# risc0/zeth

Hardware: AMD Instinct MI355X
Metric: segments/sec (higher is better)
Workload: dtype u32

## Files before the change

### zeth_amd/csrc/hash.hip

```cpp
#include "common.h"
#include "image_tree.h"
#include "poseidon2.h"
#include "poseidon2_wide.h"

using namespace zkh;

static_assert(zkh::ZKH_P2_PTAB == zkh::P2_TAB_WORDS, "common.h ZKH_P2_PTAB must equal poseidon2.h P2_TAB_WORDS");

namespace {

__global__ __launch_bounds__(256, 4) void k_hash_rows(uint32_t* __restrict__ out, const uint32_t* __restrict__ matrix,
                                                   size_t rows, uint32_t cols, const uint32_t* __restrict__ rc,
                                                   const uint32_t* __restrict__ diag) {
    const size_t r = (size_t)blockIdx.x * blockDim.x + threadIdx.x;
    if (r >= rows) return;
    uint32_t s[CELLS];
#pragma unroll
    for (int i = 0; i < CELLS; i++) s[i] = 0;
    const uint32_t* src = matrix + r;
    const uint32_t full = cols / RATE, tail = cols % RATE;
    const uint32_t blocks = full + (tail || cols == 0 ? 1u : 0u);
    for (uint32_t b = 0; b < blocks; b++) {
        const uint32_t* bsrc = src + (size_t)b * RATE * rows;
        if (b < full) {
#pragma unroll
            for (int i = 0; i < RATE; i++) s[i] = bsrc[(size_t)i * rows];
        } else {
#pragma unroll
            for (int i = 0; i < RATE; i++) s[i] = (uint32_t)i < tail ? bsrc[(size_t)i * rows] : 0u;
        }
        poseidon2_mix_sponge(s, rc, diag, b + 1 == blocks);
#pragma unroll
        for (int i = RATE; i < CELLS; i++) s[i] = p2_signed(s[i]);
    }
#pragma unroll
    for (int i = 0; i < OUT; i++) s[i] = canon((int32_t)s[RATE + i]);
    uint4* o = (uint4*)(out + r * 8);
    o[0] = make_uint4(s[0], s[1], s[2], s[3]);
    o[1] = make_uint4(s[4], s[5], s[6], s[7]);
}

__device__ __forceinline__ void fold_one(uint32_t* __restrict__ io, size_t input_size, size_t output_size, size_t i,
                                         const uint32_t* __restrict__ rc, const uint32_t* __restrict__ diag) {
    const uint4* src = (const uint4*)(io + (input_size + 2 * i) * 8);
    uint32_t s[CELLS];
    const uint4 a = src[0], b = src[1], c = src[2], d = src[3];
    s[0] = a.x; s[1] = a.y; s[2] = a.z; s[3] = a.w; s[4] = b.x; s[5] = b.y; s[6] = b.z; s[7] = b.w;
    s[8] = c.x; s[9] = c.y; s[10] = c.z; s[11] = c.w; s[12] = d.x; s[13] = d.y; s[14] = d.z; s[15] = d.w;
#pragma unroll
    for (int k = RATE; k < CELLS; k++) s[k] = 0;
    poseidon2_mix_raw<0, OUT, RATE>(s, rc, diag);
#pragma unroll
    for (int k = 0; k < OUT; k++) s[k] = p2_finish(s[k]);
    uint4* o = (uint4*)(io + (output_size + i) * 8);
    o[0] = make_uint4(s[0], s[1], s[2], s[3]);
    o[1] = make_uint4(s[4], s[5], s[6], s[7]);
}
__global__ __launch_bounds__(256, 4) void k_hash_fold(uint32_t* __restrict__ io, size_t input_size, size_t output_size,
                                                   const uint32_t* __restrict__ rc, const uint32_t* __restrict__ diag) {
    const size_t i = (size_t)blockIdx.x * blockDim.x + threadIdx.x;
    if (i >= output_size) return;
    fold_one(io, input_size, output_size, i, rc, diag);
}
__global__ __launch_bounds__(256, 4) void k_hash_fold_list(uint32_t* __restrict__ io, size_t width, const uint32_t* __restrict__ list,
                                                        const uint32_t* __restrict__ count, const uint32_t* __restrict__ rc,
                                                        const uint32_t* __restrict__ diag) {
    const uint32_t t = blockIdx.x * blockDim.x + threadIdx.x;
    if (t >= *count) return;
    fold_one(io, 2 * width, width, list[t], rc, diag);
}
__global__ __launch_bounds__(256, 4) void k_hash_walk(const uint32_t* __restrict__ list, const uint32_t* __restrict__ from, const uint32_t* __restrict__ sib,
                                                   const uint32_t* __restrict__ count, const uint32_t* __restrict__ proof, const uint32_t* __restrict__ off,
                                                   const uint32_t* __restrict__ cur, uint32_t* __restrict__ next, const uint32_t* __restrict__ rc,
                                                   const uint32_t* __restrict__ diag) {
    const uint32_t lane = blockIdx.x * blockDim.x + threadIdx.x, r = lane >> 1, v = lane & 1;
    if (r >= *count) return;
    const uint32_t item = from[r], clean = sib[r];
    const uint32_t* mine = cur + 16 * (size_t)item + 8 * v;
    const uint32_t* other = clean == 0xffffffffu ? mine + 16 : proof + *off + 8 * (size_t)clean;
    const bool odd = clean != 0xffffffffu && (list[item] & 1);
    const uint32_t* left = odd ? other : mine;
    const uint32_t* right = odd ? mine : other;
    uint32_t s[CELLS];
#pragma unroll
    for (int k = 0; k < 8; k++) { s[k] = left[k]; s[8 + k] = right[k]; }
#pragma unroll
    for (int k = RATE; k < CELLS; k++) s[k] = 0;
    poseidon2_mix_raw<0, OUT, RATE>(s, rc, diag);
#pragma unroll
    for (int k = 0; k < OUT; k++) s[k] = p2_finish(s[k]);
    uint4* o = (uint4*)(next + 16 * (size_t)r + 8 * v);
    o[0] = make_uint4(s[0], s[1], s[2], s[3]);
    o[1] = make_uint4(s[4], s[5], s[6], s[7]);
}

__device__ __forceinline__ void wide_fold_one(uint32_t* __restrict__ io, size_t input_size, size_t output_size, uint32_t gid,
                                              const uint32_t* rcs, const uint32_t* __restrict__ pc) {
    const uint32_t j = gid & 7;
    size_t parent = gid >> 3;
    const bool live = parent < output_size;
    if (!live) parent = output_size - 1;
    uint32_t c[4] = {0, 0, 0, 0};
    if (j < 4) {
        const uint4 v = *(const uint4*)(io + (input_size + 2 * parent) * 8 + 4 * j);
        c[0] = v.x; c[1] = v.y; c[2] = v.z; c[3] = v.w;
    }
    wide_permute(c, j, rcs, pc);
    if (live && j < 2) *(uint4*)(io + (output_size + parent) * 8 + 4 * j) = make_uint4(c[0], c[1], c[2], c[3]);
}
constexpr int TAIL_LOG = 7;
__global__ __launch_bounds__(8 << TAIL_LOG) void k_hash_fold_subtree(uint32_t* __restrict__ io, size_t first_parents, uint32_t levels,
                                                                     const uint32_t* __restrict__ rc, const uint32_t* __restrict__ pc) {
    __shared__ __attribute__((aligned(16))) uint32_t rcs[ROUNDS_TOTAL * CELLS + 8];
    for (uint32_t w = threadIdx.x; w < ROUNDS_TOTAL * CELLS; w += blockDim.x) rcs[w] = rc[w];
    __syncthreads();
    for (uint32_t l = 0; l < levels; l++) {
        const size_t parents = first_parents >> l;
        const uint32_t local = (1u << TAIL_LOG) >> l;
        if ((threadIdx.x >> 6) * 8 < local) {
            const uint32_t grp = threadIdx.x >> 3;
            const uint32_t gid = grp < local ? (uint32_t)((blockIdx.x * local + grp) * 8 + (threadIdx.x & 7)) : 0xffffffffu;
            wide_fold_one(io, 2 * parents, parents, gid, rcs, pc);
        }
        __threadfence_block();
        __syncthreads();
    }
}
__global__ __launch_bounds__(8 << TAIL_LOG) void k_hash_fold_tail(uint32_t* __restrict__ io, size_t first_parents,
                                                                  const uint32_t* __restrict__ rc, const uint32_t* __restrict__ pc) {
    __shared__ __attribute__((aligned(16))) uint32_t rcs[ROUNDS_TOTAL * CELLS + 8];
    for (uint32_t w = threadIdx.x; w < ROUNDS_TOTAL * CELLS; w += blockDim.x) rcs[w] = rc[w];
    __syncthreads();
    for (size_t parents = first_parents; parents >= 1; parents >>= 1) {
        if ((threadIdx.x >> 6) * 8 < parents)
            wide_fold_one(io, 2 * parents, parents, threadIdx.x, rcs, pc);
        __threadfence_block();
        __syncthreads();
    }
}

__global__ __launch_bounds__(256) void k_poseidon2_mix(uint32_t* __restrict__ io, size_t count, const uint32_t* __restrict__ rc,
                                                       const uint32_t* __restrict__ diag) {
    const size_t i = (size_t)blockIdx.x * blockDim.x + threadIdx.x;
    if (i >= count) return;
    uint4* p = (uint4*)(io + i * CELLS);
    uint32_t s[CELLS];
#pragma unroll
    for (int q = 0; q < CELLS / 4; q++) { const uint4 v = p[q]; s[4 * q] = v.x; s[4 * q + 1] = v.y; s[4 * q + 2] = v.z; s[4 * q + 3] = v.w; }
    poseidon2_mix(s, rc, diag);
#pragma unroll
    for (int q = 0; q < CELLS / 4; q++) p[q] = make_uint4(s[4 * q], s[4 * q + 1], s[4 * q + 2], s[4 * q + 3]);
}

}

extern "C" const char* zkh_poseidon2_mix(zkh_ctx* c, zkh_buf* states, size_t count) {
    ZKH_REQUIRE(states && states->len == count * CELLS, "poseidon2_mix: buffer is not count x 24 words");
    if (!count) return nullptr;
    bind_thread(c);
    k_poseidon2_mix<<<(unsigned)((count + 255) / 256), 256, 0, c->stream>>>(states->ptr(), count, c->tab.rc, c->tab.diag);
    return last_launch_error("poseidon2_mix");
}
extern "C" const char* zkh_hash_rows(zkh_ctx* c, zkh_buf* out, const zkh_buf* matrix) {
    ZKH_REQUIRE(out->len % 8 == 0 && out->len, "hash_rows: output is not a digest array");
    const size_t rows = out->len / 8;
    ZKH_REQUIRE(matrix->len % rows == 0, "hash_rows: matrix size %zu not a multiple of rows %zu", matrix->len, rows);
    const size_t cols = matrix->len / rows;
    ProfScope prof(c, "hash_rows", 4.0 * matrix->len + 32.0 * rows);
    k_hash_rows<<<(unsigned)((rows + 255) / 256), 256, 0, c->stream>>>(out->ptr(), matrix->ptr(), rows, (uint32_t)cols,
                                                                      c->tab.rc, c->tab.diag);
    return last_launch_error("hash_rows");
}
extern "C" const char* zkh_hash_fold(zkh_ctx* c, zkh_buf* io, size_t input_size, size_t output_size) {
    ZKH_REQUIRE(io->len % 8 == 0, "hash_fold: not a digest array");
    ZKH_REQUIRE((input_size + 2 * output_size) * 8 <= io->len && output_size * 2 <= input_size, "hash_fold: ranges out of bounds");
    if (!output_size) return nullptr;
    ProfScope prof(c, "hash_fold", 96.0 * output_size);
    k_hash_fold<<<(unsigned)((output_size + 255) / 256), 256, 0, c->stream>>>(io->ptr(), input_size, output_size, c->tab.rc,
                                                                             c->tab.diag);
    return last_launch_error("hash_fold");
}
extern "C" const char* zkh_merkle_fold_all(zkh_ctx* c, zkh_buf* nodes, size_t rows) {
    ZKH_REQUIRE(nodes->len == rows * 16 && rows && (rows & (rows - 1)) == 0, "merkle_fold_all: nodes must hold 2*rows digests");
    return merkle_fold_from(c, nodes, rows);
}
extern "C" const char* zkh_merkle_build(zkh_ctx* c, zkh_buf* nodes, const zkh_buf* matrix, size_t rows) {
    ZKH_REQUIRE(nodes && matrix && nodes->len == rows * 16 && rows && (rows & (rows - 1)) == 0, "merkle_build: nodes must hold 2*rows digests");
    ZKH_REQUIRE(matrix->len % rows == 0, "merkle_build: matrix size %zu not a multiple of rows %zu", matrix->len, rows);
    zkh_buf* leaves = nullptr;
    ZKH_TRY(zkh_slice(nodes, rows * 8, rows * 8, &leaves));
    const char* err = zkh_hash_rows(c, leaves, matrix);
    zkh_release(leaves);
    ZKH_TRY(err);
    return merkle_fold_from(c, nodes, rows);
}
const char* zkh::merkle_fold_from(zkh_ctx* c, zkh_buf* nodes, size_t first_layer) {
    for (size_t layer = first_layer; layer >= 2; layer /= 2) {
        const size_t parents = layer / 2;
        if (parents > ((size_t)1 << WIDE_LOG)) {
            ZKH_TRY(zkh_hash_fold(c, nodes, layer, parents));
        } else if (parents > ((size_t)1 << TAIL_LOG)) {
            uint32_t levels = 0;
            while ((parents >> levels) > ((size_t)1 << TAIL_LOG)) levels++;
            ProfScope prof(c, "hash_fold_wide", 96.0 * (2 * parents - (parents >> (levels - 1))));
            k_hash_fold_subtree<<<(unsigned)(parents >> TAIL_LOG), 8 << TAIL_LOG, 0, c->stream>>>(nodes->ptr(), parents, levels, c->tab.rc,
                                                                                                   c->tab.diag);
            ZKH_TRY(last_launch_error("hash_fold_wide"));
            layer >>= (levels - 1);
        } else {
            ProfScope prof(c, "hash_fold_tail", 96.0 * (2 * parents - 1));
            k_hash_fold_tail<<<1, 8 << TAIL_LOG, 0, c->stream>>>(nodes->ptr(), parents, c->tab.rc, c->tab.diag);
            ZKH_TRY(last_launch_error("hash_fold_tail"));
            break;
        }
    }
    return nullptr;
}
const char* zkh::hash_fold_listed(zkh_ctx* c, zkh_buf* nodes, size_t width, const uint32_t* list, const uint32_t* count, uint32_t bound) {
    ZKH_REQUIRE(bound && bound <= width && 32 * width <= nodes->len, "hash_fold_listed: %u parents of %zu in %zu words", bound, width, nodes->len);
    ProfScope prof(c, "image_sparse", 100.0 * bound);
    k_hash_fold_list<<<(bound + 255) / 256, 256, 0, c->stream>>>(nodes->ptr(), width, list, count, c->tab.rc, c->tab.diag);
    return last_launch_error("image_sparse");
}
const char* zkh::hash_walk_layer(zkh_ctx* c, const uint32_t* list, const uint32_t* from, const uint32_t* sib, const uint32_t* count, const uint32_t* proof,
                                 const uint32_t* off, const uint32_t* cur, uint32_t* next, uint32_t bound) {
    ZKH_REQUIRE(bound && bound <= 0x7fffffffu, "hash_walk_layer: %u parents", bound);
    ProfScope prof(c, "walk_hash", 200.0 * bound);
    k_hash_walk<<<(unsigned)((2 * (size_t)bound + 255) / 256), 256, 0, c->stream>>>(list, from, sib, count, proof, off, cur, next, c->tab.rc, c->tab.diag);
    return last_launch_error("walk_hash");
}
```

### zeth_amd/csrc/ntt.hip

```cpp
#include "common.h"
#include "ntt_lazy.h"

using namespace zkh;

namespace {

constexpr int NTT_THREADS = 256;

struct PassParams {
    const uint32_t* in;
    uint32_t* out;
    size_t in_col_stride;
    size_t out_col_stride;
    uint32_t log_n;
    uint32_t L, R;
    uint32_t log_t;
    uint32_t expand_bits;
    uint32_t first_layer;
    uint32_t twiddle;
    uint32_t scale;
    uint32_t zk_shift;
    const uint32_t* tile_tw;
    const uint32_t* layer_tw;
    const uint32_t* tw_lo;
    const uint32_t* tw_hi;
    const uint32_t* sh_lo;
    const uint32_t* sh_hi;
    uint32_t tiles_per_col;
    uint32_t lazy;
    uint32_t lazy_comp;
    uint32_t shift16[16];
};

template <bool INVERSE>
__global__ __launch_bounds__(NTT_THREADS) void k_ntt_pass(PassParams p) {
    extern __shared__ __attribute__((aligned(16))) uint32_t tile[];
    const uint32_t T = 1u << p.log_t, rows = 1u << p.R, elems = rows << p.log_t;
    const uint32_t tid = threadIdx.x;
    const uint32_t tile_id = xcd_remap(blockIdx.x, p.tiles_per_col);
    const uint32_t col = blockIdx.y;
    const uint32_t ltiles = 1u << (p.L - p.log_t);
    const uint32_t a = tile_id >> (p.L - p.log_t), lt = tile_id & (ltiles - 1);
    const size_t base = ((size_t)a << (p.L + p.R)) + ((size_t)lt << p.log_t);
    const uint32_t l0 = lt << p.log_t;
    const uint32_t* in = p.in + (size_t)col * p.in_col_stride;
    uint32_t* out = p.out + (size_t)col * p.out_col_stride;
    const uint32_t tw_shift = MAX_LOG_N - (p.L + p.R);
    const uint32_t pad_mask = INVERSE ? 0u : (1u << p.expand_bits) - (1u << (p.first_layer - 1));

    for (uint32_t e = tid; e < elems; e += NTT_THREADS) {
        const uint32_t m = e >> p.log_t, t = e & (T - 1);
        const size_t gi = base + ((size_t)m << p.L) + t;
        uint32_t v = (gi & pad_mask) ? 0u : in[gi >> p.expand_bits];
        if (!INVERSE && p.twiddle) {
            const uint32_t r = __brev(m) >> (32 - p.R);
            const uint32_t ex = ((l0 + t) * r) << tw_shift;
            const uint32_t w = mul_mod(p.tw_lo[ex & (TW_SIZE - 1)], p.tw_hi[ex >> TW_BITS]);
            v = mul_mod(v, w);
        }
        tile[e] = v;
    }
    __syncthreads();

    const uint32_t half_elems = elems >> 1;
    if (INVERSE) {
        for (uint32_t j = p.R; j >= 1; j--) {
            const uint32_t hb = j - 1;
            for (uint32_t q = tid; q < half_elems; q += NTT_THREADS) {
                const uint32_t t = q & (T - 1), mm = q >> p.log_t;
                const uint32_t low = mm & ((1u << hb) - 1), m = ((mm >> hb) << j) | low;
                const uint32_t i0 = (m << p.log_t) | t, i1 = i0 + (1u << (hb + p.log_t));
                const uint32_t x = tile[i0], y = tile[i1];
                const uint32_t w = p.tile_tw[low << (LDS_TW_LOG - j)];
                tile[i0] = add_mod(x, y);
                tile[i1] = mul_mod(x - y + P, w);
            }
            __syncthreads();
        }
    } else {
        for (uint32_t j = p.first_layer; j <= p.R; j++) {
            const uint32_t hb = j - 1;
            for (uint32_t q = tid; q < half_elems; q += NTT_THREADS) {
                const uint32_t t = q & (T - 1), mm = q >> p.log_t;
                const uint32_t low = mm & ((1u << hb) - 1), m = ((mm >> hb) << j) | low;
                const uint32_t i0 = (m << p.log_t) | t, i1 = i0 + (1u << (hb + p.log_t));
                const uint32_t w = p.tile_tw[low << (LDS_TW_LOG - j)];
                const uint32_t x = tile[i0], y = mul_mod(tile[i1], w);
                tile[i0] = add_mod(x, y);
                tile[i1] = sub_mod(x, y);
            }
            __syncthreads();
        }
    }

    for (uint32_t e = tid; e < elems; e += NTT_THREADS) {
        const uint32_t m = e >> p.log_t, t = e & (T - 1);
        const size_t gi = base + ((size_t)m << p.L) + t;
        uint32_t v = tile[e];
        if (INVERSE) {
            if (p.twiddle) {
                const uint32_t r = __brev(m) >> (32 - p.R);
                const uint32_t ex = ((l0 + t) * r) << tw_shift;
                const uint32_t w = mul_mod(p.tw_lo[ex & (TW_SIZE - 1)], p.tw_hi[ex >> TW_BITS]);
                v = mul_mod(v, w);
            }
            if (p.scale) v = mul_mod(v, p.scale);
            if (p.zk_shift) {
                const uint32_t pos = (uint32_t)gi;
                const uint32_t ex = __brev(pos) >> (32 - p.log_n);
                v = mul_mod(v, mul_mod(p.sh_lo[ex & (TW_SIZE - 1)], p.sh_hi[ex >> TW_BITS]));
            }
        }
        out[gi] = v;
    }
}

template <int R, bool INVERSE>
__global__ __launch_bounds__(256) void k_ntt_top(PassParams p) {
    constexpr int N = 1 << R;
    const uint32_t j0 = (blockIdx.x * 256u + threadIdx.x) << 2;
    const uint32_t* in = p.in + (size_t)blockIdx.y * p.in_col_stride + j0;
    uint32_t* out = p.out + (size_t)blockIdx.y * p.out_col_stride + j0;
    const uint32_t tw_shift = MAX_LOG_N - p.log_n;
    uint32_t v[N][4];
#pragma unroll
    for (int m = 0; m < N; m++) {
        const uint4 w = *(const uint4*)(in + ((size_t)m << p.L));
        v[m][0] = w.x; v[m][1] = w.y; v[m][2] = w.z; v[m][3] = w.w;
    }
    auto root = [&](uint32_t e) -> uint32_t {
        const uint32_t ex = e << tw_shift;
        return mul_mod(p.tw_lo[ex & (TW_SIZE - 1)], p.tw_hi[ex >> TW_BITS]);
    };
    auto four_step = [&]() {
        const uint32_t step = root(1u);
        uint32_t g = root(j0);
#pragma unroll
        for (int c = 0; c < 4; c++) {
            uint32_t pw[N];
            pw[1] = g;
#pragma unroll
            for (int r = 2; r < N; r++) pw[r] = mul_mod(pw[r - 1], g);
#pragma unroll
            for (int m = 1; m < N; m++) {
                const int r = (int)(__builtin_bitreverse32((uint32_t)m) >> (32 - R));
                v[m][c] = mul_mod(v[m][c], pw[r]);
            }
            if (c < 3) g = mul_mod(g, step);
        }
    };
    if (!INVERSE) {
        four_step();
#pragma unroll
        for (int j = 1; j <= R; j++) {
            const int hb = j - 1;
#pragma unroll
            for (int i0 = 0; i0 < N; i0++) {
                if (i0 & (1 << hb)) continue;
                const int low = i0 & ((1 << hb) - 1), i1 = i0 + (1 << hb);
                const uint32_t w = low ? p.tile_tw[(uint32_t)low << (LDS_TW_LOG - j)] : 0u;
#pragma unroll
                for (int c = 0; c < 4; c++) {
                    const uint32_t x = v[i0][c], y = low ? mul_mod(v[i1][c], w) : v[i1][c];
                    v[i0][c] = add_mod(x, y);
                    v[i1][c] = sub_mod(x, y);
                }
            }
        }
    } else {
#pragma unroll
        for (int j = R; j >= 1; j--) {
            const int hb = j - 1;
#pragma unroll
            for (int i0 = 0; i0 < N; i0++) {
                if (i0 & (1 << hb)) continue;
                const int low = i0 & ((1 << hb) - 1), i1 = i0 + (1 << hb);
                const uint32_t w = low ? p.tile_tw[(uint32_t)low << (LDS_TW_LOG - j)] : 0u;
#pragma unroll
                for (int c = 0; c < 4; c++) {
                    const uint32_t x = v[i0][c], y = v[i1][c];
                    v[i0][c] = add_mod(x, y);
                    v[i1][c] = low ? mul_mod(x - y + P, w) : sub_mod(x, y);
                }
            }
        }
        four_step();
    }
#pragma unroll
    for (int m = 0; m < N; m++) *(uint4*)(out + ((size_t)m << p.L)) = make_uint4(v[m][0], v[m][1], v[m][2], v[m][3]);
}

__global__ void k_zk_shift(uint32_t* io, size_t total, uint32_t log_n, const uint32_t* sh_lo, const uint32_t* sh_hi) {
    size_t i = (size_t)blockIdx.x * blockDim.x + threadIdx.x;
    if (i >= total) return;
    const uint32_t pos = (uint32_t)(i & (((size_t)1 << log_n) - 1));
    const uint32_t ex = log_n ? __brev(pos) >> (32 - log_n) : 0;
// ... 7 lines not shown
    const uint32_t mid = blockIdx.x;
    const uint32_t rmid = mid_bits ? __brev(mid) >> (32 - mid_bits) : 0;
    if (rmid < mid) return;
    uint32_t* col = io + (size_t)blockIdx.y * col_stride;
    const uint32_t H = 1u << BR_H;
    for (uint32_t e = threadIdx.x; e < H * H; e += blockDim.x) {
        const uint32_t hi = e >> BR_H, lo = e & (H - 1);
        ta[e] = col[((size_t)hi << (log_n - BR_H)) | ((size_t)mid << BR_H) | lo];
        if (rmid != mid) tb[e] = col[((size_t)hi << (log_n - BR_H)) | ((size_t)rmid << BR_H) | lo];
    }
    __syncthreads();
    for (uint32_t e = threadIdx.x; e < H * H; e += blockDim.x) {
        const uint32_t hi2 = e >> BR_H, lo2 = e & (H - 1);
        const uint32_t shi = __brev(lo2) >> (32 - BR_H), slo = __brev(hi2) >> (32 - BR_H);
        const uint32_t src = (shi << BR_H) | slo;
        col[((size_t)hi2 << (log_n - BR_H)) | ((size_t)rmid << BR_H) | lo2] = ta[src];
        if (rmid != mid) col[((size_t)hi2 << (log_n - BR_H)) | ((size_t)mid << BR_H) | lo2] = tb[src];
    }
}
__global__ void k_bit_reverse_small(uint32_t* io, uint32_t log_n, size_t count) {
    size_t g = (size_t)blockIdx.x * blockDim.x + threadIdx.x;
    size_t n = (size_t)1 << log_n;
    if (g >= n * count) return;
    uint32_t i = (uint32_t)(g & (n - 1));
    uint32_t r = log_n ? __brev(i) >> (32 - log_n) : 0;
    if (i < r) {
        uint32_t* col = io + (g - i);
        uint32_t x = col[i], y = col[r];
        col[i] = y; col[r] = x;
    }
}


template <int LOGR, bool INVERSE, bool BASE0, int J_LO, bool LAZY = false>
__device__ __forceinline__ void radix_layers(uint32_t (&v)[1 << LOGR], const uint32_t* __restrict__ ltab,
                                             const uint32_t base_low, const int first_b) {
    constexpr int N = 1 << LOGR;
    if (!INVERSE && LAZY) {
        lazy_layers<LOGR, BASE0, J_LO>(v, ltab, base_low, first_b);
    } else if (INVERSE) {
#pragma unroll
        for (int b = LOGR - 1; b >= 0; b--) {
            const uint32_t* tw = ltab + (1u << (J_LO + b - 1));
#pragma unroll
            for (int kk = 0; kk < (1 << b); kk++) {
                const bool unit = BASE0 && kk == 0;
                const uint32_t w = unit ? 0u : tw[base_low + ((uint32_t)kk << (J_LO - 1))];
#pragma unroll
                for (int hi = 0; hi < (N >> (b + 1)); hi++) {
                    const int k = (hi << (b + 1)) | kk;
                    const uint32_t x = v[k], y = v[k + (1 << b)];
                    v[k] = add_mod(x, y);
                    v[k + (1 << b)] = unit ? sub_mod(x, y) : mul_mod(x - y + P, w);
                }
            }
        }
    } else {
#pragma unroll
        for (int b = 0; b < LOGR; b++) {
            if (b < first_b) continue;
            const uint32_t* tw = ltab + (1u << (J_LO + b - 1));
#pragma unroll
            for (int kk = 0; kk < (1 << b); kk++) {
                const bool unit = BASE0 && kk == 0;
                const uint32_t w = unit ? 0u : tw[base_low + ((uint32_t)kk << (J_LO - 1))];
#pragma unroll
                for (int hi = 0; hi < (N >> (b + 1)); hi++) {
                    const int k = (hi << (b + 1)) | kk;
                    const uint32_t x = v[k], y = unit ? v[k + (1 << b)] : mul_mod(v[k + (1 << b)], w);
                    v[k] = add_mod(x, y);
                    v[k + (1 << b)] = sub_mod(x, y);
                }
            }
        }
    }
}

template <bool INVERSE, bool LAZY = false>
__global__ __launch_bounds__(256) void k_ntt_low12(PassParams p) {
    __shared__ __attribute__((aligned(16))) uint32_t lds[4096];
    const uint32_t tid = threadIdx.x;
    const uint32_t tile = xcd_remap(blockIdx.x, p.tiles_per_col);
    const size_t base = (size_t)tile << 12;
    const uint32_t* in = p.in + (size_t)blockIdx.y * p.in_col_stride;
    uint32_t* out = p.out + (size_t)blockIdx.y * p.out_col_stride;
    const uint32_t* __restrict__ ltab = p.layer_tw;
    const uint32_t hi = tid >> 4, low = tid & 15;
    uint32_t v[16];
    if (INVERSE) {
#pragma unroll
        for (int k = 0; k < 16; k++) v[k] = in[base + k * 256 + tid];
        radix_layers<4, true, false, 9>(v, ltab, tid, 0);
#pragma unroll
        for (int k = 0; k < 16; k++) lds[k * 256 + tid] = v[k];
        __syncthreads();
#pragma unroll
        for (int k = 0; k < 16; k++) v[k] = lds[hi * 256 + k * 16 + low];
        radix_layers<4, true, false, 5>(v, ltab, low, 0);
#pragma unroll
        for (int k = 0; k < 16; k++) lds[hi * 256 + k * 16 + low] = v[k];
        __syncthreads();
#pragma unroll
        for (int q = 0; q < 4; q++) {
            const uint4 w = ((const uint4*)lds)[tid * 4 + q];
            v[4 * q] = w.x; v[4 * q + 1] = w.y; v[4 * q + 2] = w.z; v[4 * q + 3] = w.w;
        }
        radix_layers<4, true, true, 1>(v, ltab, 0, 0);
        const size_t pos0 = base + (size_t)tid * 16;
        if (p.zk_shift) {
            const uint32_t ex = __brev((uint32_t)pos0) >> (32 - p.log_n);
            const uint32_t b = mul_mod(p.sh_lo[ex & (TW_SIZE - 1)], p.sh_hi[ex >> TW_BITS]);
#pragma unroll
            for (int k = 0; k < 16; k++) v[k] = mul_mod(mul_mod(v[k], b), p.shift16[k]);
        } else if (p.scale) {
#pragma unroll
            for (int k = 0; k < 16; k++) v[k] = mul_mod(v[k], p.scale);
        }
#pragma unroll
        for (int q = 0; q < 4; q++) ((uint4*)(out + pos0))[q] = make_uint4(v[4 * q], v[4 * q + 1], v[4 * q + 2], v[4 * q + 3]);
    } else {
        const size_t pos0 = base + (size_t)tid * 16;
        if (p.expand_bits == 0) {
#pragma unroll
            for (int q = 0; q < 4; q++) {
                const uint4 w = ((const uint4*)(in + pos0))[q];
                v[4 * q] = w.x; v[4 * q + 1] = w.y; v[4 * q + 2] = w.z; v[4 * q + 3] = w.w;
            }
        } else if (p.expand_bits == 2) {
            const uint4 w = *(const uint4*)(in + (pos0 >> 2));
            v[0] = v[1] = v[2] = v[3] = w.x; v[4] = v[5] = v[6] = v[7] = w.y;
            v[8] = v[9] = v[10] = v[11] = w.z; v[12] = v[13] = v[14] = v[15] = w.w;
        } else {
#pragma unroll
            for (int k = 0; k < 16; k++) v[k] = in[(pos0 + k) >> p.expand_bits];
        }
        radix_layers<4, false, true, 1, LAZY>(v, ltab, 0, (int)p.expand_bits);
#pragma unroll
        for (int q = 0; q < 4; q++) ((uint4*)lds)[tid * 4 + q] = make_uint4(v[4 * q], v[4 * q + 1], v[4 * q + 2], v[4 * q + 3]);
        __syncthreads();
#pragma unroll
        for (int k = 0; k < 16; k++) v[k] = lds[hi * 256 + k * 16 + low];
        radix_layers<4, false, false, 5, LAZY>(v, ltab, low, 0);
#pragma unroll
        for (int k = 0; k < 16; k++) lds[hi * 256 + k * 16 + low] = v[k];
        __syncthreads();
#pragma unroll
        for (int k = 0; k < 16; k++) v[k] = lds[k * 256 + tid];
        radix_layers<4, false, false, 9, LAZY>(v, ltab, tid, 0);
#pragma unroll
        for (int k = 0; k < 16; k++) out[base + k * 256 + tid] = v[k];
    }
}

template <int RH, bool INVERSE, bool LAZY = false>
__global__ __launch_bounds__(1 << RH) void k_ntt_high(PassParams p) {
    constexpr int LT = 4;
    constexpr uint32_t TW = 1u << LT;
    extern __shared__ __attribute__((aligned(16))) uint32_t lds[];
    const uint32_t tid = threadIdx.x, t = tid & (TW - 1), g = tid >> LT;
    const uint32_t tile_id = xcd_remap(blockIdx.x, p.tiles_per_col), col = blockIdx.y;
    const uint32_t lt_bits = p.L - LT;
    const uint32_t a = tile_id >> lt_bits, lt = tile_id & ((1u << lt_bits) - 1);
    const size_t base = ((size_t)a << (p.L + RH)) + ((size_t)lt << LT);
    const uint32_t lcol = (lt << LT) + t;
    const uint32_t tw_shift = MAX_LOG_N - (p.L + RH);
    const char* in = (const char*)(p.in + (size_t)col * p.in_col_stride + base);
    char* out = (char*)(p.out + (size_t)col * p.out_col_stride + base);
    const uint32_t tb = t * 4u;
#define TILE_IN(row) (*(const uint32_t*)(in + ((((uint32_t)(row)) << (p.L + 2)) + tb)))
#define TILE_OUT(row) (*(uint32_t*)(out + ((((uint32_t)(row)) << (p.L + 2)) + tb)))
    const uint32_t* __restrict__ ltab = p.layer_tw;
    auto tmul = [](uint32_t x, uint32_t y) -> uint32_t {
        return (LAZY && !INVERSE) ? (uint32_t)smont((int32_t)x, (int32_t)y) : mul_mod(x, y);
    };
    auto root = [&](uint32_t e) -> uint32_t {
        const uint32_t ex = e << tw_shift;
        return tmul(p.tw_lo[ex & (TW_SIZE - 1)], p.tw_hi[ex >> TW_BITS]);
    };
    uint32_t tw[16];
    if (RH == 10) {
        uint32_t w0 = root(lcol * (__brev(g) >> 26));
        if (LAZY) w0 = tmul(w0, p.lazy_comp);
        const uint32_t u1 = root(lcol * 64u), v1 = root(lcol * 256u);
        const uint32_t u2 = tmul(u1, u1), u3 = tmul(u2, u1), v2 = tmul(v1, v1), v3 = tmul(v2, v1);
        const uint32_t wi[4] = {w0, tmul(w0, u2), tmul(w0, u1), tmul(w0, u3)};
#pragma unroll
        for (int i = 0; i < 4; i++) {
            tw[4 * i] = wi[i]; tw[4 * i + 1] = tmul(wi[i], v2); tw[4 * i + 2] = tmul(wi[i], v1); tw[4 * i + 3] = tmul(wi[i], v3);
        }
    } else {
        uint32_t w0 = root(lcol * (__brev(g) >> 28));
        if (LAZY) w0 = tmul(w0, p.lazy_comp);
        const uint32_t q1 = root(lcol * 16u);
        uint32_t qp[16];
        qp[0] = w0;
#pragma unroll
        for (int e = 1; e < 16; e++) qp[e] = tmul(qp[e - 1], q1);
#pragma unroll
        for (int k = 0; k < 16; k++) tw[k] = qp[__builtin_bitreverse8((unsigned char)k) >> 4];
    }
    uint32_t v[16];
    if (RH == 10) {
        const uint32_t hi = g >> 2, low = g & 3;
        if (INVERSE) {
#pragma unroll
            for (int k = 0; k < 16; k++) v[k] = TILE_IN(k * 64 + g);
            radix_layers<4, true, false, 7>(v, ltab, g, 0);
#pragma unroll
            for (int k = 0; k < 16; k++) lds[(k * 64 + g) * TW + t] = v[k];
            __syncthreads();
#pragma unroll
            for (int k = 0; k < 16; k++) v[k] = lds[(hi * 64 + k * 4 + low) * TW + t];
            radix_layers<4, true, false, 3>(v, ltab, low, 0);
#pragma unroll
            for (int k = 0; k < 16; k++) lds[(hi * 64 + k * 4 + low) * TW + t] = v[k];
            __syncthreads();
#pragma unroll
            for (int i = 0; i < 4; i++) {
                uint32_t u[4];
                const uint32_t m0 = (g * 4 + i) * 4;
#pragma unroll
                for (int k = 0; k < 4; k++) u[k] = lds[(m0 + k) * TW + t];
                radix_layers<2, true, true, 1>(u, ltab, 0, 0);
#pragma unroll
                for (int k = 0; k < 4; k++) {
                    uint32_t x = mul_mod(u[k], tw[4 * i + k]);
                    if (p.scale) x = mul_mod(x, p.scale);
                    TILE_OUT(m0 + k) = x;
                }
            }
        } else {
#pragma unroll
            for (int i = 0; i < 4; i++) {
                uint32_t u[4];
                const uint32_t m0 = (g * 4 + i) * 4;
#pragma unroll
                for (int k = 0; k < 4; k++) {
                    const uint32_t x = TILE_IN(m0 + k);
                    u[k] = LAZY ? (uint32_t)smont((int32_t)x, (int32_t)tw[4 * i + k]) : mul_mod(x, tw[4 * i + k]);
                }
                radix_layers<2, false, true, 1, LAZY>(u, ltab, 0, 0);
#pragma unroll
                for (int k = 0; k < 4; k++) lds[(m0 + k) * TW + t] = u[k];
            }
            __syncthreads();
#pragma unroll
            for (int k = 0; k < 16; k++) v[k] = lds[(hi * 64 + k * 4 + low) * TW + t];
            radix_layers<4, false, false, 3, LAZY>(v, ltab, low, 0);
#pragma unroll
            for (int k = 0; k < 16; k++) lds[(hi * 64 + k * 4 + low) * TW + t] = v[k];
            __syncthreads();
#pragma unroll
            for (int k = 0; k < 16; k++) v[k] = lds[(k * 64 + g) * TW + t];
            radix_layers<4, false, false, 7, LAZY>(v, ltab, g, 0);
#pragma unroll
            for (int k = 0; k < 16; k++) TILE_OUT(k * 64 + g) = LAZY ? canon((int32_t)v[k]) : v[k];
        }
    } else {
        if (INVERSE) {
#pragma unroll
            for (int k = 0; k < 16; k++) v[k] = TILE_IN(k * 16 + g);
            radix_layers<4, true, false, 5>(v, ltab, g, 0);
#pragma unroll
            for (int k = 0; k < 16; k++) lds[(k * 16 + g) * TW + t] = v[k];
            __syncthreads();
#pragma unroll
            for (int k = 0; k < 16; k++) v[k] = lds[(g * 16 + k) * TW + t];
            radix_layers<4, true, true, 1>(v, ltab, 0, 0);
#pragma unroll
            for (int k = 0; k < 16; k++) {
                uint32_t x = mul_mod(v[k], tw[k]);
                if (p.scale) x = mul_mod(x, p.scale);
                TILE_OUT(g * 16 + k) = x;
            }
        } else {
#pragma unroll
            for (int k = 0; k < 16; k++) {
                const uint32_t x = TILE_IN(g * 16 + k);
                v[k] = LAZY ? (uint32_t)smont((int32_t)x, (int32_t)tw[k]) : mul_mod(x, tw[k]);
            }
            radix_layers<4, false, true, 1, LAZY>(v, ltab, 0, 0);
#pragma unroll
            for (int k = 0; k < 16; k++) lds[(g * 16 + k) * TW + t] = v[k];
            __syncthreads();
#pragma unroll
            for (int k = 0; k < 16; k++) v[k] = lds[(k * 16 + g) * TW + t];
            radix_layers<4, false, false, 5, LAZY>(v, ltab, g, 0);
#pragma unroll
            for (int k = 0; k < 16; k++) TILE_OUT(k * 16 + g) = LAZY ? canon((int32_t)v[k]) : v[k];
        }
    }
}
#undef TILE_IN
#undef TILE_OUT

struct Pass { uint32_t L, R; };
std::vector<Pass> plan_passes(uint32_t log_n) {
    std::vector<Pass> v;
    if (log_n <= 12) { v.push_back({0, log_n}); return v; }
    if (log_n < 18) {
        const uint32_t low = (log_n + 1) / 2;
        v.push_back({0, low});
        v.push_back({low, log_n - low});
        return v;
    }
    const uint32_t rem = log_n - 12;
    v.push_back({0, 12});
    if (rem == 8 || rem == 10 || rem <= 7) v.push_back({12, rem});
    else if (rem == 9) { v.push_back({12, 8}); v.push_back({20, 1}); }
    else if (rem == 11 || rem == 12) { v.push_back({12, 8}); v.push_back({20, rem - 8}); }
    else { v.push_back({12, 10}); v.push_back({22, rem - 10}); }
    return v;
}

const char* run_transform(zkh_ctx* c, bool inverse, const uint32_t* in, size_t in_col_stride, uint32_t* out,
                          size_t out_col_stride, uint32_t log_n, size_t count, uint32_t expand_bits, bool zk, const char* name) {
    ZKH_REQUIRE(log_n <= (uint32_t)MAX_LOG_N, "%s: transform size 2^%u exceeds the supported 2^%d", name, log_n, MAX_LOG_N);
    ZKH_REQUIRE(count <= 65535, "%s: too many columns (%zu)", name, count);
    std::vector<Pass> passes = plan_passes(log_n);
    const size_t n = (size_t)1 << log_n;
    Fp ninv = fp_inv(fp_encode((uint32_t)(n % P)));
    const size_t npass = passes.size();
    const bool lazy = !inverse && npass == 2 && passes[0].R == 12 && (passes[1].R == 8 || passes[1].R == 10) && expand_bits <= 4;
    const uint32_t lazy_reds = lazy ? lazy_reductions(4, expand_bits) + 2 * lazy_reductions(4, 0) + lazy_reductions(passes[1].R, 0) : 0;
    const uint32_t lazy_comp = lazy ? fp_pow(Fp::raw(R2), lazy_reds).v : 0;
    for (size_t pi = 0; pi < npass; pi++) {
        const Pass ps = inverse ? passes[npass - 1 - pi] : passes[pi];
        PassParams p{};
        const bool first = pi == 0, last = pi + 1 == npass;
        p.in = first ? in : out;
        p.in_col_stride = first ? in_col_stride : out_col_stride;
        p.out = out; p.out_col_stride = out_col_stride;
        p.log_n = log_n; p.L = ps.L; p.R = ps.R;
        const bool reg_high = ps.L >= 4 && (ps.R == 8 || ps.R == 10);
        p.log_t = ps.L == 0 ? 0 : (ps.L < 4 ? ps.L : 4);
        if (ps.L != 0 && !reg_high && ps.R < 12) p.log_t = std::max<uint32_t>(p.log_t, std::min<uint32_t>(ps.L, 12 - ps.R));
        while (p.R + p.log_t > 14 && p.log_t > 0) p.log_t--;
        p.expand_bits = (!inverse && first) ? expand_bits : 0;
        p.first_layer = (!inverse && first) ? std::min(expand_bits, ps.R) + 1 : 1;
        p.twiddle = ps.L != 0;
        p.scale = (inverse && last) ? ninv.v : 0;
        p.zk_shift = (inverse && last && zk) ? 1 : 0;
        p.lazy = lazy; p.lazy_comp = lazy_comp;
        p.tile_tw = inverse ? c->tab.tile_rev : c->tab.tile_fwd;
        p.layer_tw = inverse ? c->tab.layer_rev : (lazy ? c->tab.layer_fwd_lazy : c->tab.layer_fwd);
        p.tw_lo = inverse ? c->tab.tw_rev_lo : c->tab.tw_fwd_lo;
        p.tw_hi = inverse ? c->tab.tw_rev_hi : c->tab.tw_fwd_hi;
        p.sh_lo = c->tab.shift_lo; p.sh_hi = c->tab.shift_hi;
        if (p.zk_shift && log_n >= 4) {
            const Fp three = fp_encode(3);
            for (uint32_t k = 0; k < 16; k++)
                p.shift16[k] = (ninv * fp_pow(three, (uint64_t)(bitrev32(k) >> 28) << (log_n - 4))).v;
        }
        p.tiles_per_col = (uint32_t)(n >> (p.R + p.log_t));
        const size_t lds = ((size_t)4 << (p.R + p.log_t));
        dim3 grid(p.tiles_per_col, (unsigned)count);
        const double alg_bytes = pi == 0 ? 4.0 * count * (double)(((size_t)1 << log_n) >> expand_bits) + 4.0 * count * (double)n : 0.0;
        const bool scale_here = p.scale != 0;
        const bool k_low = ps.L == 0 && ps.R == 12 && p.expand_bits <= 4;
        const bool k_h10 = !k_low && ps.L >= 4 && p.log_t == 4 && ps.R == 10 && !(scale_here && p.zk_shift);
        const bool k_h8 = !k_low && !k_h10 && ps.L >= 4 && p.log_t == 4 && ps.R == 8 && !(scale_here && p.zk_shift);
        const bool k_top = !k_low && !k_h10 && !k_h8 && ps.L >= 12 && ps.L + ps.R == log_n && ps.R >= 1 && ps.R <= 4 && p.twiddle &&
                           p.expand_bits == 0 && p.first_layer == 1 && !scale_here && !p.zk_shift;
        const std::string pname = std::string(name) + (k_low ? ":k_ntt_low12" : k_h10 ? ":k_ntt_high10" : k_h8 ? ":k_ntt_high8" : k_top ? ":k_ntt_top" : ":k_ntt_pass");
        ProfScope prof(c, pname.c_str(), alg_bytes);
        if (ps.L == 0 && ps.R == 12 && p.expand_bits <= 4) {
            if (inverse) k_ntt_low12<true><<<grid, 256, 0, c->stream>>>(p);
            else if (lazy) k_ntt_low12<false, true><<<grid, 256, 0, c->stream>>>(p);
            else k_ntt_low12<false><<<grid, 256, 0, c->stream>>>(p);
        } else if (ps.L >= 4 && p.log_t == 4 && ps.R == 10 && !(scale_here && p.zk_shift)) {
            if (inverse) k_ntt_high<10, true><<<grid, 1024, lds, c->stream>>>(p);
            else if (lazy) k_ntt_high<10, false, true><<<grid, 1024, lds, c->stream>>>(p);
// ... 89 lines not shown
```

Measured before the change: 43.66.

## Switch hash and NTT global accesses to AMDGPU buffer resource loads/stores

```diff
diff --git a/zeth_amd/csrc/bufaddr.h b/zeth_amd/csrc/bufaddr.h
--- /dev/null
+++ b/zeth_amd/csrc/bufaddr.h
@@ -0,0 +1,64 @@
+#pragma once
+#include <cstdint>
+
+#if defined(__HIPCC__) || defined(__CUDACC__)
+#define ZKH_BUF_HD __host__ __device__
+#else
+#define ZKH_BUF_HD
+#endif
+
+namespace zkh {
+
+constexpr uint64_t BUF_MAX_EXTENT = 0xffffffffull;
+constexpr uint64_t BUF_WINDOW = 1ull << 31;
+
+struct BufSpan {
+    uint64_t base;
+    uint32_t extent;
+};
+
+ZKH_BUF_HD constexpr BufSpan buf_span(uint64_t base, uint64_t end, uint64_t advance) {
+    const uint64_t b = base + advance, left = end - b;
+    const uint32_t hi = (uint32_t)(left >> 32), lo = (uint32_t)left;
+    return BufSpan{b, hi == 0 ? lo : ((int32_t)hi < 0 ? 0u : (uint32_t)BUF_MAX_EXTENT)};
+}
+ZKH_BUF_HD constexpr bool buf_fits(uint64_t step_bytes, uint64_t steps, uint64_t window) {
+    return step_bytes != 0 && window <= BUF_MAX_EXTENT + 1 && steps <= window / step_bytes;
+}
+
+#if defined(__HIPCC__)
+using buf_rsrc = __amdgpu_buffer_rsrc_t;
+typedef uint32_t buf_u32x2 __attribute__((ext_vector_type(2)));
+typedef uint32_t buf_u32x4 __attribute__((ext_vector_type(4)));
+
+__device__ __forceinline__ buf_rsrc buf_make(const BufSpan s) {
+    return __builtin_amdgcn_make_buffer_rsrc((void*)s.base, (short)0, (int)s.extent, 0x00020000);
+}
+__device__ __forceinline__ buf_rsrc buf_make(const void* base, uint32_t bytes) { return buf_make(BufSpan{(uint64_t)base, bytes}); }
+template <uint32_t IMM = 0>
+__device__ __forceinline__ uint32_t buf_load_b32(buf_rsrc r, uint32_t voff, uint32_t soff = 0) {
+    return __builtin_amdgcn_raw_buffer_load_b32(r, (int)(voff + IMM), (int)soff, 0);
+}
+template <uint32_t IMM = 0>
+__device__ __forceinline__ buf_u32x2 buf_load_b64(buf_rsrc r, uint32_t voff, uint32_t soff = 0) {
+    return __builtin_amdgcn_raw_buffer_load_b64(r, (int)(voff + IMM), (int)soff, 0);
+}
+template <uint32_t IMM = 0>
+__device__ __forceinline__ buf_u32x4 buf_load_b128(buf_rsrc r, uint32_t voff, uint32_t soff = 0) {
+    return __builtin_amdgcn_raw_buffer_load_b128(r, (int)(voff + IMM), (int)soff, 0);
+}
+template <uint32_t IMM = 0>
+__device__ __forceinline__ void buf_store_b32(buf_rsrc r, uint32_t v, uint32_t voff, uint32_t soff = 0) {
+    __builtin_amdgcn_raw_buffer_store_b32(v, r, (int)(voff + IMM), (int)soff, 0);
+}
+template <uint32_t IMM = 0>
+__device__ __forceinline__ void buf_store_b64(buf_rsrc r, buf_u32x2 v, uint32_t voff, uint32_t soff = 0) {
+    __builtin_amdgcn_raw_buffer_store_b64(v, r, (int)(voff + IMM), (int)soff, 0);
+}
+template <uint32_t IMM = 0>
+__device__ __forceinline__ void buf_store_b128(buf_rsrc r, buf_u32x4 v, uint32_t voff, uint32_t soff = 0) {
+    __builtin_amdgcn_raw_buffer_store_b128(v, r, (int)(voff + IMM), (int)soff, 0);
+}
+#endif
+
+}
diff --git a/zeth_amd/csrc/hash.hip b/zeth_amd/csrc/hash.hip
--- a/zeth_amd/csrc/hash.hip
+++ b/zeth_amd/csrc/hash.hip
@@ -1,4 +1,5 @@
 #include "common.h"
+#include "bufaddr.h"
 #include "image_tree.h"
 #include "poseidon2.h"
 #include "poseidon2_wide.h"
@@ -9,6 +10,7 @@
 
 namespace {
 
+template <bool PER_COLUMN>
 __global__ __launch_bounds__(256, 4) void k_hash_rows(uint32_t* __restrict__ out, const uint32_t* __restrict__ matrix,
                                                    size_t rows, uint32_t cols, const uint32_t* __restrict__ rc,
                                                    const uint32_t* __restrict__ diag) {
@@ -17,17 +19,23 @@
     uint32_t s[CELLS];
 #pragma unroll
     for (int i = 0; i < CELLS; i++) s[i] = 0;
-    const uint32_t* src = matrix + r;
+    const uint32_t voff = (uint32_t)r * 4u;
+    const uint64_t col_bytes = (uint64_t)rows * 4u, mbase = (uint64_t)matrix, mend = mbase + (uint64_t)cols * col_bytes;
     const uint32_t full = cols / RATE, tail = cols % RATE;
     const uint32_t blocks = full + (tail || cols == 0 ? 1u : 0u);
     for (uint32_t b = 0; b < blocks; b++) {
-        const uint32_t* bsrc = src + (size_t)b * RATE * rows;
+        const uint64_t bbase = mbase + (uint64_t)b * RATE * col_bytes;
+        const buf_rsrc bsrc = buf_make(buf_span(bbase, mend, 0));
+        auto column = [&](int i) -> uint32_t {
+            if (PER_COLUMN) return buf_load_b32(buf_make(buf_span(bbase, mend, (uint64_t)i * col_bytes)), voff);
+            return buf_load_b32(bsrc, voff, (uint32_t)i * (uint32_t)col_bytes);
+        };
         if (b < full) {
 #pragma unroll
-            for (int i = 0; i < RATE; i++) s[i] = bsrc[(size_t)i * rows];
+            for (int i = 0; i < RATE; i++) s[i] = column(i);
         } else {
 #pragma unroll
-            for (int i = 0; i < RATE; i++) s[i] = (uint32_t)i < tail ? bsrc[(size_t)i * rows] : 0u;
+            for (int i = 0; i < RATE; i++) s[i] = (uint32_t)i < tail ? column(i) : 0u;
         }
         poseidon2_mix_sponge(s, rc, diag, b + 1 == blocks);
 #pragma unroll
@@ -35,16 +43,18 @@
     }
 #pragma unroll
     for (int i = 0; i < OUT; i++) s[i] = canon((int32_t)s[RATE + i]);
-    uint4* o = (uint4*)(out + r * 8);
-    o[0] = make_uint4(s[0], s[1], s[2], s[3]);
-    o[1] = make_uint4(s[4], s[5], s[6], s[7]);
-}
-
-__device__ __forceinline__ void fold_one(uint32_t* __restrict__ io, size_t input_size, size_t output_size, size_t i,
+    const size_t r0 = (size_t)blockIdx.x * blockDim.x;
+    const uint32_t left = (uint32_t)rows - (uint32_t)r0;
+    const buf_rsrc o = buf_make(out + r0 * 8, (left < 256 ? left : 256) * 32);
+    const uint32_t ooff = threadIdx.x * 32u;
+    buf_store_b128(o, buf_u32x4{s[0], s[1], s[2], s[3]}, ooff);
+    buf_store_b128<16>(o, buf_u32x4{s[4], s[5], s[6], s[7]}, ooff);
+}
+
+__device__ __forceinline__ void fold_one(const buf_rsrc in, uint32_t ioff, const buf_rsrc out, uint32_t ooff,
                                          const uint32_t* __restrict__ rc, const uint32_t* __restrict__ diag) {
-    const uint4* src = (const uint4*)(io + (input_size + 2 * i) * 8);
-    uint32_t s[CELLS];
-    const uint4 a = src[0], b = src[1], c = src[2], d = src[3];
+    uint32_t s[CELLS];
+    const buf_u32x4 a = buf_load_b128(in, ioff), b = buf_load_b128<16>(in, ioff), c = buf_load_b128<32>(in, ioff), d = buf_load_b128<48>(in, ioff);
     s[0] = a.x; s[1] = a.y; s[2] = a.z; s[3] = a.w; s[4] = b.x; s[5] = b.y; s[6] = b.z; s[7] = b.w;
     s[8] = c.x; s[9] = c.y; s[10] = c.z; s[11] = c.w; s[12] = d.x; s[13] = d.y; s[14] = d.z; s[15] = d.w;
 #pragma unroll
@@ -52,22 +62,25 @@
     poseidon2_mix_raw<0, OUT, RATE>(s, rc, diag);
 #pragma unroll
     for (int k = 0; k < OUT; k++) s[k] = p2_finish(s[k]);
-    uint4* o = (uint4*)(io + (output_size + i) * 8);
-    o[0] = make_uint4(s[0], s[1], s[2], s[3]);
-    o[1] = make_uint4(s[4], s[5], s[6], s[7]);
+    buf_store_b128(out, buf_u32x4{s[0], s[1], s[2], s[3]}, ooff);
+    buf_store_b128<16>(out, buf_u32x4{s[4], s[5], s[6], s[7]}, ooff);
 }
 __global__ __launch_bounds__(256, 4) void k_hash_fold(uint32_t* __restrict__ io, size_t input_size, size_t output_size,
                                                    const uint32_t* __restrict__ rc, const uint32_t* __restrict__ diag) {
-    const size_t i = (size_t)blockIdx.x * blockDim.x + threadIdx.x;
-    if (i >= output_size) return;
-    fold_one(io, input_size, output_size, i, rc, diag);
+    const size_t i0 = (size_t)blockIdx.x * blockDim.x;
+    if (i0 + threadIdx.x >= output_size) return;
+    const uint32_t left = (uint32_t)output_size - (uint32_t)i0;
+    const uint32_t mine = left < 256 ? left : 256;
+    fold_one(buf_make(io + (input_size + 2 * i0) * 8, mine * 64), threadIdx.x * 64u, buf_make(io + (output_size + i0) * 8, mine * 32),
+             threadIdx.x * 32u, rc, diag);
 }
 __global__ __launch_bounds__(256, 4) void k_hash_fold_list(uint32_t* __restrict__ io, size_t width, const uint32_t* __restrict__ list,
                                                         const uint32_t* __restrict__ count, const uint32_t* __restrict__ rc,
                                                         const uint32_t* __restrict__ diag) {
     const uint32_t t = blockIdx.x * blockDim.x + threadIdx.x;
     if (t >= *count) return;
-    fold_one(io, 2 * width, width, list[t], rc, diag);
+    const uint32_t i = list[t];
+    fold_one(buf_make(io + 2 * width * 8, (uint32_t)width * 64), i * 64u, buf_make(io + width * 8, (uint32_t)width * 32), i * 32u, rc, diag);
 }
 __global__ __launch_bounds__(256, 4) void k_hash_walk(const uint32_t* __restrict__ list, const uint32_t* __restrict__ from, const uint32_t* __restrict__ sib,
                                                    const uint32_t* __restrict__ count, const uint32_t* __restrict__ proof, const uint32_t* __restrict__ off,
@@ -152,6 +165,15 @@
     for (int q = 0; q < CELLS / 4; q++) p[q] = make_uint4(s[4 * q], s[4 * q + 1], s[4 * q + 2], s[4 * q + 3]);
 }
 
+uint64_t buf_window() {
+    const char* v = getenv("ZKH_BUF_WINDOW");
+    const char* armed = getenv("ZKH_TEST_HOOKS");
+    if (!v || !*v || !armed || strcmp(armed, "1") != 0) return BUF_WINDOW;
+    char* end = nullptr;
+    const unsigned long long w = strtoull(v, &end, 10);
+    return (end && *end == 0 && w >= 4 && w <= BUF_WINDOW) ? w : BUF_WINDOW;
+}
+
 }
 
 extern "C" const char* zkh_poseidon2_mix(zkh_ctx* c, zkh_buf* states, size_t count) {
@@ -166,9 +188,14 @@
     const size_t rows = out->len / 8;
     ZKH_REQUIRE(matrix->len % rows == 0, "hash_rows: matrix size %zu not a multiple of rows %zu", matrix->len, rows);
     const size_t cols = matrix->len / rows;
+    ZKH_REQUIRE(rows <= ((size_t)1 << MAX_LOG_N), "hash_rows: %zu rows exceed the supported 2^%d", rows, MAX_LOG_N);
     ProfScope prof(c, "hash_rows", 4.0 * matrix->len + 32.0 * rows);
-    k_hash_rows<<<(unsigned)((rows + 255) / 256), 256, 0, c->stream>>>(out->ptr(), matrix->ptr(), rows, (uint32_t)cols,
-                                                                      c->tab.rc, c->tab.diag);
+    if (buf_fits(4 * (uint64_t)rows, RATE, buf_window()))
+        k_hash_rows<false><<<(unsigned)((rows + 255) / 256), 256, 0, c->stream>>>(out->ptr(), matrix->ptr(), rows, (uint32_t)cols,
+                                                                                 c->tab.rc, c->tab.diag);
+    else
+        k_hash_rows<true><<<(unsigned)((rows + 255) / 256), 256, 0, c->stream>>>(out->ptr(), matrix->ptr(), rows, (uint32_t)cols,
+                                                                                c->tab.rc, c->tab.diag);
     return last_launch_error("hash_rows");
 }
 extern "C" const char* zkh_hash_fold(zkh_ctx* c, zkh_buf* io, size_t input_size, size_t output_size) {
@@ -218,6 +245,7 @@
 }
 const char* zkh::hash_fold_listed(zkh_ctx* c, zkh_buf* nodes, size_t width, const uint32_t* list, const uint32_t* count, uint32_t bound) {
     ZKH_REQUIRE(bound && bound <= width && 32 * width <= nodes->len, "hash_fold_listed: %u parents of %zu in %zu words", bound, width, nodes->len);
+    ZKH_REQUIRE(width <= ((size_t)1 << (MAX_LOG_N - 1)), "hash_fold_listed: a layer of %zu parents exceeds the supported 2^%d", width, MAX_LOG_N - 1);
     ProfScope prof(c, "image_sparse", 100.0 * bound);
     k_hash_fold_list<<<(bound + 255) / 256, 256, 0, c->stream>>>(nodes->ptr(), width, list, count, c->tab.rc, c->tab.diag);
     return last_launch_error("image_sparse");
diff --git a/zeth_amd/csrc/ntt.hip b/zeth_amd/csrc/ntt.hip
--- a/zeth_amd/csrc/ntt.hip
+++ b/zeth_amd/csrc/ntt.hip
@@ -1,4 +1,5 @@
 #include "common.h"
+#include "bufaddr.h"
 #include "ntt_lazy.h"
 
 using namespace zkh;
@@ -41,17 +42,17 @@
     const uint32_t col = blockIdx.y;
     const uint32_t ltiles = 1u << (p.L - p.log_t);
     const uint32_t a = tile_id >> (p.L - p.log_t), lt = tile_id & (ltiles - 1);
-    const size_t base = ((size_t)a << (p.L + p.R)) + ((size_t)lt << p.log_t);
+    const uint32_t base = (a << (p.L + p.R)) + (lt << p.log_t);
     const uint32_t l0 = lt << p.log_t;
-    const uint32_t* in = p.in + (size_t)col * p.in_col_stride;
-    uint32_t* out = p.out + (size_t)col * p.out_col_stride;
+    const buf_rsrc in = buf_make(p.in + (size_t)col * p.in_col_stride, 4u << (p.log_n - p.expand_bits));
+    const buf_rsrc out = buf_make(p.out + (size_t)col * p.out_col_stride, 4u << p.log_n);
     const uint32_t tw_shift = MAX_LOG_N - (p.L + p.R);
     const uint32_t pad_mask = INVERSE ? 0u : (1u << p.expand_bits) - (1u << (p.first_layer - 1));
 
     for (uint32_t e = tid; e < elems; e += NTT_THREADS) {
         const uint32_t m = e >> p.log_t, t = e & (T - 1);
-        const size_t gi = base + ((size_t)m << p.L) + t;
-        uint32_t v = (gi & pad_mask) ? 0u : in[gi >> p.expand_bits];
+        const uint32_t gi = base + (m << p.L) + t;
+        uint32_t v = (gi & pad_mask) ? 0u : buf_load_b32(in, (gi >> p.expand_bits) * 4u);
         if (!INVERSE && p.twiddle) {
             const uint32_t r = __brev(m) >> (32 - p.R);
             const uint32_t ex = ((l0 + t) * r) << tw_shift;
@@ -95,7 +96,7 @@
 
     for (uint32_t e = tid; e < elems; e += NTT_THREADS) {
         const uint32_t m = e >> p.log_t, t = e & (T - 1);
-        const size_t gi = base + ((size_t)m << p.L) + t;
+        const uint32_t ti = (m << p.L) + t, gi = base + ti;
         uint32_t v = tile[e];
         if (INVERSE) {
             if (p.twiddle) {
@@ -106,12 +107,12 @@
             }
             if (p.scale) v = mul_mod(v, p.scale);
             if (p.zk_shift) {
-                const uint32_t pos = (uint32_t)gi;
+                const uint32_t pos = gi;
                 const uint32_t ex = __brev(pos) >> (32 - p.log_n);
                 v = mul_mod(v, mul_mod(p.sh_lo[ex & (TW_SIZE - 1)], p.sh_hi[ex >> TW_BITS]));
             }
         }
-        out[gi] = v;
+        buf_store_b32(out, v, ti * 4u, base * 4u);
     }
 }
 
@@ -285,14 +286,15 @@
     const uint32_t tid = threadIdx.x;
     const uint32_t tile = xcd_remap(blockIdx.x, p.tiles_per_col);
     const size_t base = (size_t)tile << 12;
-    const uint32_t* in = p.in + (size_t)blockIdx.y * p.in_col_stride;
-    uint32_t* out = p.out + (size_t)blockIdx.y * p.out_col_stride;
+    const buf_rsrc in = buf_make(p.in + (size_t)blockIdx.y * p.in_col_stride + (base >> p.expand_bits), 16384u >> p.expand_bits);
+    const buf_rsrc out = buf_make(p.out + (size_t)blockIdx.y * p.out_col_stride + base, 16384u);
+    const uint32_t strided = tid * 4u, run = tid * 64u;
     const uint32_t* __restrict__ ltab = p.layer_tw;
     const uint32_t hi = tid >> 4, low = tid & 15;
     uint32_t v[16];
     if (INVERSE) {
 #pragma unroll
-        for (int k = 0; k < 16; k++) v[k] = in[base + k * 256 + tid];
+        for (int k = 0; k < 16; k++) v[k] = buf_load_b32(in, strided, k * 1024u);
         radix_layers<4, true, false, 9>(v, ltab, tid, 0);
 #pragma unroll
         for (int k = 0; k < 16; k++) lds[k * 256 + tid] = v[k];
@@ -309,9 +311,9 @@
             v[4 * q] = w.x; v[4 * q + 1] = w.y; v[4 * q + 2] = w.z; v[4 * q + 3] = w.w;
         }
         radix_layers<4, true, true, 1>(v, ltab, 0, 0);
-        const size_t pos0 = base + (size_t)tid * 16;
+        const uint32_t pos0 = (uint32_t)base + tid * 16;
         if (p.zk_shift) {
-            const uint32_t ex = __brev((uint32_t)pos0) >> (32 - p.log_n);
+            const uint32_t ex = __brev(pos0) >> (32 - p.log_n);
             const uint32_t b = mul_mod(p.sh_lo[ex & (TW_SIZE - 1)], p.sh_hi[ex >> TW_BITS]);
 #pragma unroll
             for (int k = 0; k < 16; k++) v[k] = mul_mod(mul_mod(v[k], b), p.shift16[k]);
@@ -319,23 +321,22 @@
 #pragma unroll
             for (int k = 0; k < 16; k++) v[k] = mul_mod(v[k], p.scale);
         }
-#pragma unroll
-        for (int q = 0; q < 4; q++) ((uint4*)(out + pos0))[q] = make_uint4(v[4 * q], v[4 * q + 1], v[4 * q + 2], v[4 * q + 3]);
+        buf_store_b128<0>(out, buf_u32x4{v[0], v[1], v[2], v[3]}, run);
+        buf_store_b128<16>(out, buf_u32x4{v[4], v[5], v[6], v[7]}, run);
+        buf_store_b128<32>(out, buf_u32x4{v[8], v[9], v[10], v[11]}, run);
+        buf_store_b128<48>(out, buf_u32x4{v[12], v[13], v[14], v[15]}, run);
     } else {
-        const size_t pos0 = base + (size_t)tid * 16;
         if (p.expand_bits == 0) {
-#pragma unroll
-            for (int q = 0; q < 4; q++) {
-                const uint4 w = ((const uint4*)(in + pos0))[q];
-                v[4 * q] = w.x; v[4 * q + 1] = w.y; v[4 * q + 2] = w.z; v[4 * q + 3] = w.w;
-            }
+            const buf_u32x4 w0 = buf_load_b128<0>(in, run), w1 = buf_load_b128<16>(in, run), w2 = buf_load_b128<32>(in, run), w3 = buf_load_b128<48>(in, run);
+            v[0] = w0.x; v[1] = w0.y; v[2] = w0.z; v[3] = w0.w; v[4] = w1.x; v[5] = w1.y; v[6] = w1.z; v[7] = w1.w;
+            v[8] = w2.x; v[9] = w2.y; v[10] = w2.z; v[11] = w2.w; v[12] = w3.x; v[13] = w3.y; v[14] = w3.z; v[15] = w3.w;
         } else if (p.expand_bits == 2) {
-            const uint4 w = *(const uint4*)(in + (pos0 >> 2));
+            const buf_u32x4 w = buf_load_b128(in, tid * 16u);
             v[0] = v[1] = v[2] = v[3] = w.x; v[4] = v[5] = v[6] = v[7] = w.y;
             v[8] = v[9] = v[10] = v[11] = w.z; v[12] = v[13] = v[14] = v[15] = w.w;
         } else {
 #pragma unroll
-            for (int k = 0; k < 16; k++) v[k] = in[(pos0 + k) >> p.expand_bits];
+            for (int k = 0; k < 16; k++) v[k] = buf_load_b32(in, ((tid * 16 + k) >> p.expand_bits) * 4u);
         }
         radix_layers<4, false, true, 1, LAZY>(v, ltab, 0, (int)p.expand_bits);
 #pragma unroll
@@ -351,7 +352,7 @@
         for (int k = 0; k < 16; k++) v[k] = lds[k * 256 + tid];
         radix_layers<4, false, false, 9, LAZY>(v, ltab, tid, 0);
 #pragma unroll
-        for (int k = 0; k < 16; k++) out[base + k * 256 + tid] = v[k];
+        for (int k = 0; k < 16; k++) buf_store_b32(out, v[k], strided, k * 1024u);
     }
 }
 
@@ -367,11 +368,12 @@
     const size_t base = ((size_t)a << (p.L + RH)) + ((size_t)lt << LT);
     const uint32_t lcol = (lt << LT) + t;
     const uint32_t tw_shift = MAX_LOG_N - (p.L + RH);
-    const char* in = (const char*)(p.in + (size_t)col * p.in_col_stride + base);
-    char* out = (char*)(p.out + (size_t)col * p.out_col_stride + base);
-    const uint32_t tb = t * 4u;
-#define TILE_IN(row) (*(const uint32_t*)(in + ((((uint32_t)(row)) << (p.L + 2)) + tb)))
-#define TILE_OUT(row) (*(uint32_t*)(out + ((((uint32_t)(row)) << (p.L + 2)) + tb)))
+    const uint32_t tile_bytes = (((1u << RH) - 1u) << (p.L + 2)) + 4u * TW;
+    const buf_rsrc in = buf_make(p.in + (size_t)col * p.in_col_stride + base, tile_bytes);
+    const buf_rsrc out = buf_make(p.out + (size_t)col * p.out_col_stride + base, tile_bytes);
+    const uint32_t rows1 = (g << (p.L + 2)) + t * 4u, rows16 = (g << (p.L + 6)) + t * 4u;
+#define TILE_IN(lane_rows, row) buf_load_b32(in, lane_rows, (uint32_t)(row) << (p.L + 2))
+#define TILE_OUT(lane_rows, row, x) buf_store_b32(out, x, lane_rows, (uint32_t)(row) << (p.L + 2))
     const uint32_t* __restrict__ ltab = p.layer_tw;
     auto tmul = [](uint32_t x, uint32_t y) -> uint32_t {
         return (LAZY && !INVERSE) ? (uint32_t)smont((int32_t)x, (int32_t)y) : mul_mod(x, y);
@@ -407,7 +409,7 @@
         const uint32_t hi = g >> 2, low = g & 3;
         if (INVERSE) {
 #pragma unroll
-            for (int k = 0; k < 16; k++) v[k] = TILE_IN(k * 64 + g);
+            for (int k = 0; k < 16; k++) v[k] = TILE_IN(rows1, k * 64);
             radix_layers<4, true, false, 7>(v, ltab, g, 0);
 #pragma unroll
             for (int k = 0; k < 16; k++) lds[(k * 64 + g) * TW + t] = v[k];
@@ -429,7 +431,7 @@
                 for (int k = 0; k < 4; k++) {
                     uint32_t x = mul_mod(u[k], tw[4 * i + k]);
                     if (p.scale) x = mul_mod(x, p.scale);
-                    TILE_OUT(m0 + k) = x;
+                    TILE_OUT(rows16, i * 4 + k, x);
                 }
             }
         } else {
@@ -439,7 +441,7 @@
                 const uint32_t m0 = (g * 4 + i) * 4;
 #pragma unroll
                 for (int k = 0; k < 4; k++) {
-                    const uint32_t x = TILE_IN(m0 + k);
+                    const uint32_t x = TILE_IN(rows16, i * 4 + k);
                     u[k] = LAZY ? (uint32_t)smont((int32_t)x, (int32_t)tw[4 * i + k]) : mul_mod(x, tw[4 * i + k]);
                 }
                 radix_layers<2, false, true, 1, LAZY>(u, ltab, 0, 0);
@@ -457,12 +459,12 @@
             for (int k = 0; k < 16; k++) v[k] = lds[(k * 64 + g) * TW + t];
             radix_layers<4, false, false, 7, LAZY>(v, ltab, g, 0);
 #pragma unroll
-            for (int k = 0; k < 16; k++) TILE_OUT(k * 64 + g) = LAZY ? canon((int32_t)v[k]) : v[k];
+            for (int k = 0; k < 16; k++) TILE_OUT(rows1, k * 64, LAZY ? canon((int32_t)v[k]) : v[k]);
         }
     } else {
         if (INVERSE) {
 #pragma unroll
-            for (int k = 0; k < 16; k++) v[k] = TILE_IN(k * 16 + g);
+            for (int k = 0; k < 16; k++) v[k] = TILE_IN(rows1, k * 16);
             radix_layers<4, true, false, 5>(v, ltab, g, 0);
 #pragma unroll
             for (int k = 0; k < 16; k++) lds[(k * 16 + g) * TW + t] = v[k];
@@ -474,12 +476,12 @@
             for (int k = 0; k < 16; k++) {
                 uint32_t x = mul_mod(v[k], tw[k]);
                 if (p.scale) x = mul_mod(x, p.scale);
-                TILE_OUT(g * 16 + k) = x;
+                TILE_OUT(rows16, k, x);
             }
         } else {
 #pragma unroll
             for (int k = 0; k < 16; k++) {
-                const uint32_t x = TILE_IN(g * 16 + k);
+                const uint32_t x = TILE_IN(rows16, k);
                 v[k] = LAZY ? (uint32_t)smont((int32_t)x, (int32_t)tw[k]) : mul_mod(x, tw[k]);
             }
             radix_layers<4, false, true, 1, LAZY>(v, ltab, 0, 0);
@@ -490,7 +492,7 @@
             for (int k = 0; k < 16; k++) v[k] = lds[(k * 16 + g) * TW + t];
             radix_layers<4, false, false, 5, LAZY>(v, ltab, g, 0);
 #pragma unroll
-            for (int k = 0; k < 16; k++) TILE_OUT(k * 16 + g) = LAZY ? canon((int32_t)v[k]) : v[k];
+            for (int k = 0; k < 16; k++) TILE_OUT(rows1, k * 16, LAZY ? canon((int32_t)v[k]) : v[k]);
         }
     }
 }
```

Measured after the change: 43.78, median of 5. About the same (+0.3%).
